# jean-pierreBoth/gsearch

Hardware: AMD Instinct MI355X
Metric: query genomes/sec (higher is better)
Workload: dtype f32

## Files before the change

### gsearch_amd/csrc/gs_index.hip

```cpp
#include <algorithm>
#include <functional>
#include <chrono>
#include <math.h>
#include <memory>
#include <stdlib.h>
#include <string.h>
#include <vector>
#include <sys/stat.h>
#include "gs_internal.hpp"
#include "gs_spec.hpp"
#include "gs_insert_rows.hpp"
#include "gs_hnswio_parse.hpp"

namespace gs {

constexpr int ST = 1024;
constexpr int SMAXI = 16;
constexpr int RIF = 8;
#define KEY(c, id) (((uint64_t)(c) << 32) | (uint64_t)(id))
#define KCNT(k) ((uint32_t)((k) >> 32))
#define KID(k) ((uint32_t)(k))
#define INF_CNT 0xFFFFFFFFu

struct IndexDev {
// ... 423 lines not shown
#pragma unroll
            for (int t = 0; t < 4; t++) if (top[t] && m >= (uint32_t)t) { const uint32_t c = m - t; atomicAdd(&coarse[c / HB], top[t]); if (c / HB == target) atomicAdd(&fine[c % HB], top[t]); }
        }
        __syncthreads();
        if (threadIdx.x < 64) {
            uint32_t run = 0, found = 0xFFFFFFFFu, before = 0;
            for (uint32_t b0 = 0; b0 < nb && found == 0xFFFFFFFFu; b0 += 64) {
                const uint32_t x = b0 + lane < nb ? coarse[b0 + lane] : 0;
                uint32_t inc = x;
#pragma unroll
                for (int o = 1; o < 64; o <<= 1) { const uint32_t y = __shfl_up(inc, o); if ((int)lane >= o) inc += y; }
                const uint64_t hit = __ballot(run + inc >= efs);
                if (hit) { const uint32_t l = (uint32_t)__ffsll((long long)hit) - 1; found = b0 + l; before = run + __shfl(inc, l) - __shfl(x, l); }
                run += __shfl(inc, 63);
            }
            if (lane == 0) { res[0] = found; res[1] = before; }
        }
        __syncthreads();
        const uint32_t bin = res[0], before = res[1];
        if (bin == target) {
            if (threadIdx.x == 0) { uint32_t run = before, f = 0; for (; f < (uint32_t)HB; f++) { run += fine[f]; if (run >= efs) break; } res[2] = bin * HB + f; }
            __syncthreads();
            const uint32_t tau = res[2];
            __syncthreads();
            return tau;
        }
        target = bin;
        __syncthreads();
    }
    return INF_CNT;
}

__device__ __forceinline__ uint32_t uni32(uint32_t v) { return (uint32_t)__builtin_amdgcn_readfirstlane((int)v); }
__device__ __forceinline__ uint32_t row_prefix4(uint32_t x)
{
    static_assert(DT / 64 == 8, "four wavefronts to a half of the workgroup");
    x += (uint32_t)__builtin_amdgcn_update_dpp(0, (int)x, 0x111, 0xF, 0xF, false);
    x += (uint32_t)__builtin_amdgcn_update_dpp(0, (int)x, 0x112, 0xF, 0xF, false);
    return x;
}

struct Phase2IO { uint32_t nT, evals, pops; bool tm; long long c_build, c_drain; uint64_t *wl; uint32_t cap_log, nlog; };
template <bool ONEG, bool WLOG, bool SPLIT>
__device__ __forceinline__ void dense_phase2(const IndexDev &ix, const DenseLds &S, uint32_t *vis, const uint16_t *__restrict__ matrow, uint32_t tau, uint32_t knbn,
                                                       uint64_t *Gold, uint64_t *Gnew, uint32_t headG, uint32_t nG, uint32_t headN, uint32_t nN, uint64_t Tmax, Phase2IO &io,
                                                       uint32_t vis_w, uint32_t *__restrict__ visg)
{
    const uint32_t maxdeg = 2 * ix.M;
    constexpr uint32_t CN = ONEG ? 512u : (uint32_t)DCN;
    const uint32_t wv = threadIdx.x >> 6, lane = threadIdx.x & 63;
    uint32_t nT = io.nT, st_p2 = 0;
    uint32_t *s_cnt = (uint32_t *)&S.scal[4];
    uint32_t *WL = (uint32_t *)Gnew;
    uint64_t *TA = Gold;
    if (threadIdx.x < 4) s_cnt[threadIdx.x] = threadIdx.x == 3 ? io.nlog : 0u;
    __syncthreads();
    {
        const uint64_t *src = Gold + headG;
        const uint32_t liveG = nG - headG, liveN = nN - headN;
        for (uint32_t i = threadIdx.x; i < liveG; i += DT) { const uint64_t k = src[i]; if (KCNT(k) <= tau) WL[atomicAdd(&s_cnt[0], 1u)] = KID(k); }
        for (uint32_t i = threadIdx.x; i < liveN; i += DT) { const uint64_t k = S.N[headN + i]; if (KCNT(k) <= tau) WL[atomicAdd(&s_cnt[0], 1u)] = KID(k); }
    }
    __syncthreads();
    uint32_t *bfA = (uint32_t *)S.A, *bfB = S.Eid;
    const uint32_t bytesA = 8 * maxdeg + 8 * (DWIN + 4) + 8 * (CN + 4), bytesB = (uint32_t)((uint8_t *)S.wsum - (uint8_t *)S.Eid);
    uint32_t lgA = 5, lgB = 5;
// ... 279 lines not shown
            }
        }
    }
    __syncthreads();
    for (uint32_t i0 = 0; i0 < n; i0 += NF * DT) {
        uint64_t kf[NF];
#pragma unroll
        for (int u = 0; u < NF; u++) { const uint32_t i = i0 + u * DT + threadIdx.x; kf[u] = i < n ? src[i] : ~(uint64_t)0; }
#pragma unroll
        for (int u = 0; u < NF; u++) {
            const uint64_t k = kf[u];
            const bool live = k != ~(uint64_t)0 && KCNT(k) <= dlimit;
            const bool isS = live && k < cutkey, isK = live && !isS;
            const uint64_t bS = __ballot(isS), bK = __ballot(isK);
            uint32_t baseS = 0, baseK = 0;
            if (lane == 0) { if (bS) baseS = atomicAdd(&cnt[0], (uint32_t)__popcll(bS)); if (bK) baseK = atomicAdd(&cnt[1], (uint32_t)__popcll(bK)); }
            baseS = (uint32_t)__builtin_amdgcn_readfirstlane((int)baseS); baseK = (uint32_t)__builtin_amdgcn_readfirstlane((int)baseK);
            if (isS) { const uint32_t pos = baseS + (uint32_t)__popcll(bS & ((1ull << lane) - 1)); if (pos < 64u) S.N[pos] = k; }
            if (isK) dst[baseK + (uint32_t)__popcll(bK & ((1ull << lane) - 1))] = k;
        }
    }
    __syncthreads();
    const uint32_t nsel = cnt[0] < 64u ? cnt[0] : 64u, nkeep = cnt[1];
    if (sel && wv == 0) {
        const uint64_t k = lane < nsel ? S.N[lane] : ~(uint64_t)0;
        uint32_t rank = 0;
        for (uint32_t j = 0; j < nsel; j++) rank += (S.N[j] < k);
        if (lane < nsel) S.N[64 + rank] = k;
    }
    __syncthreads();
    if (sel && wv == 0) {
        pkey = lane < nsel ? S.N[64 + lane] : ~(uint64_t)0;
        nP = nsel;
        pv = (nkeep && nsel) ? readlane_u64(pkey, (int)nsel - 1) : ~(uint64_t)0;
        if (lane < 3) S.W[fb + lane] = pkey;
    }
    if (threadIdx.x == 0) S.scal[4] = nkeep;
    stat += (sel ? 1ull : (1ull << 24)) + ((unsigned long long)rounds << 40);
    __syncthreads();
}

template <bool VLDS, bool PROF, int OCC, bool ONEG, bool WLOG, bool SPLIT = false>
__global__ __launch_bounds__(DT, OCC) void k_hnsw_search_dense(IndexDev ix, uint64_t nq, uint32_t knbn, uint32_t ef, const uint16_t *__restrict__ mat, uint64_t mat_ld,
                                                           uint32_t *__restrict__ scratch, uint32_t scratch_words, uint64_t *__restrict__ cbuf, uint32_t capC,
                                                           unsigned long long *__restrict__ counter, uint64_t *__restrict__ ids_out, float *__restrict__ dist_out,
                                                           uint32_t *__restrict__ count_out, uint64_t *__restrict__ evals_out, unsigned long long *__restrict__ prof,
                                                           unsigned long long *__restrict__ stats, uint64_t *__restrict__ wlog, uint32_t cap_log, uint32_t sort_cap,
                                                           uint64_t *__restrict__ w_out, uint32_t *__restrict__ w_n, const uint32_t *__restrict__ ep_in, uint32_t vis_w_arg)
{
    static_assert(!SPLIT || VLDS, "the split bitmap is a form of the LDS placement");
    extern __shared__ __attribute__((aligned(16))) uint8_t s_raw[];
    const uint32_t maxdeg = 2 * ix.M;
    const uint32_t efs = ef > knbn ? ef : knbn;
    const uint32_t vis_w = SPLIT ? vis_w_arg : 0u;
    const uint32_t nb = dense_nblocks(ix.m), hwords = nb * (HB / 2), vis_words = SPLIT ? (vis_w >> 5) : (uint32_t)((ix.n + 31) / 32);
    const uint32_t visg_words = SPLIT && ix.n > vis_w ? (uint32_t)((ix.n - vis_w + 31) / 32) : 0u;
    unsigned long long st_pq = 0;
    uint32_t st_pops = 0, st_acc = 0, st_p1 = 0, st_p2 = 0;
    constexpr bool PHASE2 = true;
#ifdef GS_DENSE_PQ_OFF
    constexpr bool PQ = false;
#else
    constexpr bool PQ = true;
#endif
    long long t_a = 0, t_b = 0, t_c = 0, t_d = 0, t_e = 0, n_pop = 0, n_merge = 0;
    long long tq1 = 0, tq2 = 0, tq3 = 0, tq4 = 0, tna = 0;
    constexpr uint32_t CN = ONEG ? 512u : (uint32_t)DCN;
    DenseLds S = carve_dense(s_raw, ix.m, knbn, maxdeg, SPLIT ? (uint64_t)vis_w : ix.n, VLDS, CN);
#define GS_TRAV_LOAD(p) __builtin_nontemporal_load(p)
#define GS_DROWX(K, PD, PI)                                                                                                \
    do {                                                                                                                   \
        const uint32_t rid_ = uni32(KID(K));                                                                               \
        uint32_t tx_ = threadIdx.x;                                                                                        \
        asm volatile("" : "+v"(tx_));                \
        const uint32_t hl_ = ONEG ? tx_ : tx_ & 255u, ho_ = hl_ * 4u;    \
        PD = ix.deg0[rid_];                                                                                                \
        PI = hl_ < maxdeg ? GS_TRAV_LOAD((const uint32_t *)((const uint8_t *)(ix.nbr0 + (uint64_t)rid_ * maxdeg) + ho_)) : 0; \
    } while (0)
#define GS_DROW(K) GS_DROWX(K, pdeg, pid)
    uint32_t *vis = VLDS ? S.vis : scratch + (uint64_t)blockIdx.x * scratch_words;
    Hist3 hs; hs.Hf = VLDS ? scratch + (uint64_t)blockIdx.x * scratch_words : S.Hf; hs.H2 = S.H2; hs.H1 = S.H1;
    uint32_t *visg = SPLIT ? scratch + (uint64_t)blockIdx.x * scratch_words + hwords : nullptr;
    uint64_t *Cb[2] = {cbuf + (uint64_t)blockIdx.x * 2 * capC, cbuf + (uint64_t)blockIdx.x * 2 * capC + capC};
    const uint32_t wv = threadIdx.x >> 6, lane = threadIdx.x & 63;
    const uint32_t half = ONEG ? 0u : threadIdx.x >> 8, hl = ONEG ? threadIdx.x : threadIdx.x & 255;
    for (;;) {
        __syncthreads();
        if (threadIdx.x == 0) S.scal[1] = atomicAdd(counter, 1ull);
        __syncthreads();
        const uint64_t qi = S.scal[1];
        if (qi >= nq) break;
        uint64_t *wl = WLOG ? wlog + (uint64_t)blockIdx.x * cap_log : nullptr;
        uint32_t nlog = 1;
        const uint16_t *matrow = mat + qi * mat_ld;
        const bool tm = PHASE2 && stats && blockIdx.x == 0 && threadIdx.x == 0;
        const long long tm0 = tm ? clock64() : 0;
        const uint32_t tau = PHASE2 ? dense_row_tau(matrow, ix.n, ix.m, efs, S.H1, S.hist, S.wsum) : 0u;
        const long long tm1 = tm ? clock64() : 0;
        for (uint32_t w = threadIdx.x; w < vis_words; w += DT) vis[w] = 0;
        if (SPLIT) for (uint32_t w = threadIdx.x; w < visg_words; w += DT) visg[w] = 0;
        for (uint32_t w = threadIdx.x; w < hwords; w += DT) hs.Hf[w] = 0;
        for (uint32_t w = threadIdx.x; w < nb * (HB / HG / 2); w += DT) S.H2[w] = 0;
        for (uint32_t w = threadIdx.x; w < nb; w += DT) S.H1[w] = 0;
        uint32_t evals = 1;
        uint32_t ep = (uint32_t)ix.entry, ep_cnt = matrow[ep];
        const bool given = WLOG && ep_in && ep_in[qi] != 0xFFFFFFFFu;
        if (given) { ep = ep_in[qi]; ep_cnt = matrow[ep]; evals = 0; }
        for (int L = given ? 0 : ix.top; L >= 1; L--) {
            for (;;) {
                const uint32_t *nbr; uint32_t deg;
                node_neighbours(ix, ep, L, nbr, deg);
                if (deg == 0) break;
                if (threadIdx.x == 0) S.scal[0] = ~(uint64_t)0;
                __syncthreads();
                evals += deg;
                if (threadIdx.x < deg) { const uint32_t c = matrow[nbr[threadIdx.x]]; if (c < ep_cnt) atomicMin((unsigned long long *)&S.scal[0], (unsigned long long)KEY(c, threadIdx.x)); }
// ... 40 lines not shown
                c = S.W[fb]; c1 = S.W[fb + 1]; c2 = S.W[fb + 2];
                const bool empty = c == ~(uint64_t)0, crowded = nU + maxdeg > capC && nU - nU_lc >= maxdeg;
                if (empty && nU == 0) break;
                if (empty || crowded) {
                    pq_rebuild(ix, S, Cb[cur], Cb[cur ^ 1], capC, nU, empty, full ? dmax : INF_CNT, pkey, pv, nP, fb, st_pq);
                    cur ^= 1; nU = (uint32_t)S.scal[4]; nU_lc = nU;
                    continue;
                }
                if (KCNT(c) > dmax) break;
                if (uni32(wv) == 0) {
                    pkey = wave_shl1_u64(pkey); if (lane == 63) pkey = ~(uint64_t)0;
                    nP--;
                    if (lane < 3) S.W[(fb ^ 4u) + lane] = pkey;
                }
            } else {
            if (headG < nG && headG - wbase >= wn) {
                __syncthreads();
                wbase = headG; wn = nG - headG < (uint32_t)DWIN ? nG - headG : (uint32_t)DWIN;
                if (threadIdx.x < wn + 3) S.W[threadIdx.x] = threadIdx.x < wn ? Cb[cur][headG + threadIdx.x] : ~(uint64_t)0;
                __syncthreads();
            }
            const uint32_t wo = headG - wbase;
            const uint64_t g0 = S.W[wo], g1 = S.W[wo + 1], g2 = S.W[wo + 2];
            const uint64_t n0 = S.N[headN], n1 = S.N[headN + 1], n2 = S.N[headN + 2];
            c = g0 < n0 ? g0 : n0;
            if (c == ~(uint64_t)0) break;
            if (KCNT(c) > dmax) break;
            if (g0 < n0) { headG++; c1 = g1 < n0 ? g1 : n0; c2 = g1 < n0 ? (g2 < n0 ? g2 : n0) : (g1 < n1 ? g1 : n1); }
            else { headN++; c1 = g0 < n1 ? g0 : n1; c2 = g0 < n1 ? (g1 < n1 ? g1 : n1) : (g0 < n2 ? g0 : n2); }
            }
            const long long p0 = PROF ? clock64() : 0;
            uint32_t id = 0, cntv = 0; bool unv = false, below = false;
            uint64_t bal = 0, balb = 0;
            const bool expanding = ONEG || uni32(half) == (it & 1u);
            if (expanding) {
                if (pk != c) {
                    if (ONEG && nk == c) { pid = nid; pdeg = ndeg; nk = ~(uint64_t)0; }
                    else GS_DROW(c);
                    pst = 1;
                }
                id = pid;
                if (hl < pdeg) {
                    const uint32_t bit = 1u << (id & 31);
                    uint32_t old;
                    if (SPLIT && id >= vis_w) {
                        if (pst == 2 && !pclr) old = bit;
                        else old = __hip_atomic_fetch_or(&visg[(id - vis_w) >> 5], bit, __ATOMIC_RELAXED, __HIP_MEMORY_SCOPE_WORKGROUP);
                    }
                    else if (VLDS) old = atomicOr(&vis[id >> 5], bit);
                    else old = __hip_atomic_fetch_or(&vis[id >> 5], bit, __ATOMIC_RELAXED, __HIP_MEMORY_SCOPE_WORKGROUP);
                    unv = !(old & bit);
                    if (unv) cntv = (pst == 2 && pclr) ? pcnt : (uint32_t)matrow[id];
                }
                below = unv && cntv < dmax;
                bal = __ballot(unv); balb = __ballot(below);
            } else if (!ONEG && c1 != ~(uint64_t)0) {
                if (pk != c1) {
                    pk = c1; pst = 1;
                    GS_DROW(c1);
                }
                if (VLDS) {
                    pclr = false;
                    if (hl < pdeg) {
                        if (SPLIT && pid >= vis_w) pclr = !((__hip_atomic_load(&visg[(pid - vis_w) >> 5], __ATOMIC_RELAXED, __HIP_MEMORY_SCOPE_AGENT) >> (pid & 31)) & 1u);
                        else pclr = !((vis[pid >> 5] >> (pid & 31)) & 1u);
                        if (pclr) pcnt = matrow[pid];
                    }
                    pst = 2;
                }
            } else if (!ONEG) pk = ~(uint64_t)0;
            it++;
            const long long p1 = PROF ? clock64() : 0;
            uint32_t *ws = S.wsum + ((it & 1) ? 8 : 0);
            if (expanding && lane == 0) ws[wv] = (uint32_t)__popcll(bal) | ((uint32_t)__popcll(balb) << 16);
            if (!ONEG) {
                if (expanding) {
                    pk = c2; pst = 1;
                    if (c2 != ~(uint64_t)0) GS_DROW(c2);
                }
            } else {
                pk = c1;
                if (c1 != ~(uint64_t)0) {
                    if (nk == c1) {
                        pid = nid; pdeg = ndeg; pclr = false;
                        if (VLDS) {
                            if (hl < pdeg) {
                                if (SPLIT && pid >= vis_w) pclr = !((__hip_atomic_load(&visg[(pid - vis_w) >> 5], __ATOMIC_RELAXED, __HIP_MEMORY_SCOPE_AGENT) >> (pid & 31)) & 1u);
                                else pclr = !((vis[pid >> 5] >> (pid & 31)) & 1u);
                                if (pclr) pcnt = matrow[pid];
                            }
                            pst = 2;
                        } else pst = 1;
                    } else { GS_DROW(c1); pst = 1; }
                }
                nk = c2;
                if (c2 != ~(uint64_t)0) GS_DROWX(c2, ndeg, nid);
            }
            lds_barrier();
            const long long p2 = PROF ? clock64() : 0;
            uint32_t tot = 0, pre = 0;
            if (ONEG) {
#pragma unroll
                for (int w = 0; w < DT / 64; w++) { const uint32_t x = ws[w]; tot += x; if (w < (int)wv) pre += x; }
            } else {
                const uint32_t wsw = ws[(((it & 1u) ^ 1u) << 2) + (lane & 3u)], wsum4 = row_prefix4(wsw);
                tot = (uint32_t)__builtin_amdgcn_readlane((int)wsum4, 3);
                pre = (uint32_t)__builtin_amdgcn_readlane((int)(wsum4 - wsw), (int)(uni32(wv) & 3u));
            }
            const uint32_t ne = tot & 0xFFFFu, B = tot >> 16;
            const long long p3 = PROF ? clock64() : 0;
            if (PROF && blockIdx.x == 0 && threadIdx.x == 0) { t_a += p1 - p0; t_b += p2 - p1; t_c += p3 - p2; n_pop++; }
            st_pops++;
            if (PHASE2 && dmax != tau) st_p1++;
            if (ne == 0) continue;
            evals += ne;
            bool slow;
            if (!full) slow = nR + ne > efs;
            else { if (B == 0) continue; slow = B > tieT; }
            uint64_t mykey = ~(uint64_t)0, ab; bool acc = false;
            uint32_t na, ci, aoff;
            const uint32_t off = pre & 0xFFFFu, boff = pre >> 16;
            if (!slow) { acc = below; na = B; ci = cntv; mykey = KEY(cntv, id); ab = balb; aoff = boff; }
            else {
                if (unv) { const uint32_t pos = off + (uint32_t)__popcll(bal & ((1ull << lane) - 1)); S.Eid[pos] = id; S.Ecnt[pos] = cntv; }
                const uint32_t CH = (nb + DT - 1) / DT;
                uint32_t loc = 0;
                for (uint32_t k2 = 0; k2 < CH; k2++) { const uint32_t idx = threadIdx.x * CH + k2; if (idx < nb) loc += S.H1[idx]; }
                uint32_t inc = loc;
#pragma unroll
                for (int o = 1; o < 64; o <<= 1) { const uint32_t y = __shfl_up(inc, o); if ((int)lane >= o) inc += y; }
                if (lane == 63) S.wsum[16 + wv] = inc;
                __syncthreads();
                ci = threadIdx.x < ne ? S.Ecnt[threadIdx.x] : INF_CNT;
                uint32_t woff = 0;
#pragma unroll
                for (int w = 0; w < DT / 64; w++) if (w < (int)wv) woff += S.wsum[16 + w];
                uint32_t run = woff + inc - loc;
                for (uint32_t k2 = 0; k2 < CH; k2++) { const uint32_t idx = threadIdx.x * CH + k2; if (idx < nb) { S.P1[idx] = run; run += S.H1[idx]; } }
                lds_barrier();
                if (threadIdx.x < ne && ci < dmax) {
                    uint32_t le = S.P1[ci / HB];
                    for (uint32_t g = (ci / HB) * (HB / HG); g < ci / HG; g++) le += h16(S.H2, g);
                    const uint32_t w0 = (ci / HG) * (HG / 2), w1 = ci >> 1;
                    for (uint32_t w = w0; w <= w1; w++) {
                        const uint32_t x = hf_word<VLDS>(hs.Hf, w);
                        le += x & 0xFFFFu;
                        if (w < w1 || (ci & 1)) le += x >> 16;
                    }
                    if (le < efs) {
#pragma unroll 8
                        for (uint32_t j = 0; j < threadIdx.x; j++) le += (S.Ecnt[j] <= ci);
                    }
                    acc = le < efs;
                }
                if (acc) mykey = KEY(ci, S.Eid[threadIdx.x]);
                ab = __ballot(acc);
                if (lane == 0) S.wsum[24 + wv] = (uint32_t)__popcll(ab);
                lds_barrier();
                aoff = 0; na = 0;
#pragma unroll
                for (int w = 0; w < DT / 64; w++) { const uint32_t x = S.wsum[24 + w]; if (w < (int)wv) aoff += x; na += x; }
            }
            const long long p4 = PROF ? clock64() : 0;
            if (PROF && blockIdx.x == 0 && threadIdx.x == 0) t_d += p4 - p3;
            if (na == 0) continue;
            n_merge++; st_acc++;
            uint64_t minA = 0;
            const uint32_t fbn = (it & 1u) * 4u;
            if (PQ) {
                if (acc) { hist_add<VLDS>(hs, ci, 1); S.As[aoff + (uint32_t)__popcll(ab & ((1ull << lane) - 1))] = mykey; }
                lds_barrier();
                if (uni32(wv) == 0) {
                    uint64_t tany = 0;
                    uint64_t *U = Cb[cur];
                    uint32_t nu = nU;
                    for (uint32_t b0 = 0; b0 < na; b0 += 64) {
                        const uint64_t k = b0 + lane < na ? S.As[b0 + lane] : ~(uint64_t)0;
                        tany |= __ballot(k < Tmax);
                        const bool toU = k != ~(uint64_t)0 && k >= pv;
                        const uint64_t bu = __ballot(toU);
                        if (toU) { const uint32_t pos = nu + (uint32_t)__popcll(bu & ((1ull << lane) - 1)); if (pos < capC) U[pos] = k; }
                        nu += (uint32_t)__popcll(bu);
                        uint64_t pend = __ballot(k != ~(uint64_t)0 && k < pv);
                        while (pend) {
                            const int l = __ffsll((long long)pend) - 1;
                            pend &= pend - 1;
                            const uint64_t kk = readlane_u64(k, l);
                            if (kk >= pv) { if (lane == 0 && nu < capC) U[nu] = kk; nu++; continue; }
                            const uint32_t pos = (uint32_t)__popcll(__ballot(pkey < kk));
                            const uint64_t ev = readlane_u64(pkey, 63), up = wave_shr1_u64(pkey);
                            pkey = lane < pos ? pkey : (lane == pos ? kk : up);
                            if (ev != ~(uint64_t)0) { if (lane == 0 && nu < capC) U[nu] = ev; nu++; }
                            else nP++;
                            if (nP == 64) pv = readlane_u64(pkey, 63);
                        }
                    }
                    if (lane < 3) S.W[fbn + lane] = pkey;
                    if (lane == 0) { S.scal[4] = nu; S.scal[5] = tany ? 0 : ~(uint64_t)0; }
                }
                lds_barrier();
                nU = (uint32_t)S.scal[4]; minA = S.scal[5];
            } else {
                if (acc) { hist_add<VLDS>(hs, ci, 1); S.As[aoff + (uint32_t)__popcll(ab & ((1ull << lane) - 1))] = mykey; }
                lds_barrier();
                if (threadIdx.x < na) {
                    const uint64_t k = S.As[threadIdx.x];
                    uint32_t rank = 0;
#pragma unroll 8
                    for (uint32_t j = 0; j < na; j++) rank += (S.As[j] < k);
                    S.A[rank] = k;
                }
                lds_barrier();
            }
            if (WLOG) { if (nlog + na <= cap_log && threadIdx.x < na) wl[nlog + threadIdx.x] = PQ ? S.As[threadIdx.x] : S.A[threadIdx.x]; nlog += na; }
            {
                const uint64_t a0 = PQ ? 0 : S.A[0], a1 = PQ ? 0 : (na > 1 ? S.A[1] : ~(uint64_t)0);
                const uint64_t n1 = PQ ? S.W[fbn] : (a0 < c1 ? a0 : c1);
                const uint64_t n2 = PQ ? S.W[fbn + 1] : (a0 < c1 ? (a1 < c1 ? a1 : c1) : (a0 < c2 ? a0 : c2));
                if (!ONEG) {
                    const uint64_t want = expanding ? n2 : n1;
                    if (want != ~(uint64_t)0 && pk != want) {
                        pk = want; pst = 1;
                        GS_DROW(want);
                    }
                } else {
                    if (n1 != ~(uint64_t)0 && pk != n1) {
                        const uint64_t ok = pk; const uint32_t oid = pid, odeg = pdeg;
                        if (nk == n1) { pid = nid; pdeg = ndeg; }
                        else GS_DROW(n1);
                        pk = n1; pst = 1;
                        nk = ok; nid = oid; ndeg = odeg;
                    }
                    if (n2 != ~(uint64_t)0 && nk != n2) { nk = n2; GS_DROWX(n2, ndeg, nid); }
                }
            }
            const long long q1 = PROF ? clock64() : 0;
            const uint32_t dold = dmax;
            if (nR + na >= efs) {
                const uint32_t excess = nR + na - efs;
                if (full && excess < tieT) {
                    if (threadIdx.x == 0 && excess) hist_sub<VLDS>(hs, dmax, excess);
                    tieT -= excess;
                } else {
                    __syncthreads();
                    if (threadIdx.x < 64) {
                        uint32_t d = full ? dmax : ix.m, ex = excess, tt = 0;
                        for (;;) {
                            d = hist_find_down<VLDS>(hs, d, lane, tt);
// ... 133 lines not shown
            uint32_t *cntp = (uint32_t *)s_raw;
            if (threadIdx.x == 0) cntp[0] = 0;
            __syncthreads();
            bool bad = nlog > cap_log;
            if (!bad) for (uint32_t i = threadIdx.x; i < nlog; i += DT) {
                const uint64_t k = wl[i];
                if (KCNT(k) <= dmax) { const uint32_t pos = atomicAdd(&cntp[0], 1u); if (pos < sort_cap) buf[pos] = k; }
            }
            __syncthreads();
            const uint32_t cnt = cntp[0];
            if (cnt > sort_cap) bad = true;
            if (bad) { if (threadIdx.x == 0) w_n[qi] = 0xFFFFFFFFu; }
            else {
                uint32_t n2 = 2; while (n2 < cnt) n2 <<= 1;
                for (uint32_t i = cnt + threadIdx.x; i < n2; i += DT) buf[i] = ~(uint64_t)0;
                __syncthreads();
                for (uint32_t kk = 2; kk <= n2; kk <<= 1)
                    for (uint32_t j = kk >> 1; j > 0; j >>= 1) {
                        for (uint32_t i = threadIdx.x; i < n2; i += DT) {
                            const uint32_t l = i ^ j;
                            if (l > i) {
                                const uint64_t a = buf[i], b = buf[l];
                                if ((a > b) == ((i & kk) == 0)) { buf[i] = b; buf[l] = a; }
                            }
                        }
                        __syncthreads();
                    }
                const uint32_t nW = cnt < efs ? cnt : efs;
                for (uint32_t i = threadIdx.x; i < nW; i += DT) w_out[qi * efs + i] = buf[i];
                if (threadIdx.x == 0) w_n[qi] = nW;
            }
        }
    }
#undef GS_DROW
#undef GS_DROWX
    if (stats && threadIdx.x == 0) { atomicAdd(&stats[1], (unsigned long long)st_pops); atomicAdd(&stats[2], (unsigned long long)st_acc); atomicAdd(&stats[5], (unsigned long long)st_p1); atomicAdd(&stats[6], (unsigned long long)st_p2); if (st_pq) atomicAdd(&stats[15], st_pq); }
    if (PROF && blockIdx.x == 0 && threadIdx.x == 0) {
        atomicAdd(&prof[0], (unsigned long long)t_a); atomicAdd(&prof[1], (unsigned long long)t_b); atomicAdd(&prof[2], (unsigned long long)t_c);
        atomicAdd(&prof[3], (unsigned long long)t_d); atomicAdd(&prof[4], (unsigned long long)t_e); atomicAdd(&prof[5], (unsigned long long)n_pop); atomicAdd(&prof[6], (unsigned long long)n_merge);
        atomicAdd(&prof[8], (unsigned long long)tq1); atomicAdd(&prof[9], (unsigned long long)tq2); atomicAdd(&prof[10], (unsigned long long)tq3); atomicAdd(&prof[11], (unsigned long long)tq4); atomicAdd(&prof[12], (unsigned long long)tna);
    }
}


__device__ __forceinline__ SearchLds carve_lds(uint8_t *base, uint32_t ef, uint32_t maxdeg)
{
    SearchLds S;
    const size_t capC = 2 * (size_t)ef + maxdeg + 64;
    S.R = (uint64_t *)base; base += 8 * (size_t)ef;
    S.C = (uint64_t *)base; base += 8 * capC;
    S.A = (uint64_t *)base; base += 8 * (size_t)maxdeg;
    S.As = (uint64_t *)base; base += 8 * (size_t)maxdeg;
    S.scal = (uint64_t *)base; base += 8 * 8;
    S.Eid = (uint32_t *)base; base += 4 * (size_t)maxdeg;
    S.Ecnt = (uint32_t *)base; base += 4 * (size_t)maxdeg;
    S.wsum = (uint32_t *)base;
    return S;
}

template <int KIND>
__global__ __launch_bounds__(ST) void k_hnsw_search(IndexDev ix, const uint8_t *__restrict__ queries, uint64_t nq, uint32_t knbn, uint32_t ef,
                                                     const uint16_t *__restrict__ mat, uint64_t mat_ld, uint32_t *__restrict__ visited, uint32_t vis_words, unsigned long long *__restrict__ counter,
                                                     uint64_t *__restrict__ ids_out, float *__restrict__ dist_out, uint32_t *__restrict__ count_out,
                                                     uint64_t *__restrict__ evals_out)
{
    extern __shared__ __attribute__((aligned(16))) uint8_t s_raw[];
    const uint32_t maxdeg = 2 * ix.M;
    const uint32_t efs = ef > knbn ? ef : knbn;
    SearchLds S = carve_lds(s_raw, efs, maxdeg);
// ... 830 lines not shown
{
    const size_t cap = 160 * 1024 - 1024;
    const size_t l = dense_lds_bytes(ix->prm.m, knbn, maxdeg, ix->n, true, maxdeg > (uint32_t)DT / 2 ? 512u : (uint32_t)DCN);
    const char *e = getenv("GS_DENSE_VIS");
    if (e && !strcmp(e, "global")) return false;
    if (e && !strcmp(e, "lds")) return l <= cap;
    return l <= cap;
}
static uint32_t dense_split_w(const gs_index *ix, uint32_t knbn, uint32_t maxdeg, uint32_t dcn, size_t min_bytes = 0, bool many_queries = false)
{
    const char *e = getenv("GS_DENSE_VIS");
    const bool forced = e && !strcmp(e, "split");
    if (e && !forced) { if (!strcmp(e, "global") || !strcmp(e, "lds")) return 0; }
    const bool one_per_cu = many_queries && round_up(dense_lds_bytes(ix->prm.m, knbn, maxdeg, ix->n, true, dcn), 1280) > (size_t)(160 * 1024 / 2);
    if (!forced && !one_per_cu && dense_vis_in_lds(ix, knbn, maxdeg)) return 0;
    const size_t base = std::max(dense_lds_bytes(ix->prm.m, knbn, maxdeg, 0, true, dcn), min_bytes);
    int per = getenv("GS_SPLIT_PER_CU") ? std::max(1, std::min(3, atoi(getenv("GS_SPLIT_PER_CU")))) : 2;
    uint64_t w = 0;
    for (; per >= 1 && w < 1024; per--) {
        const size_t budget = (size_t)(160 * 1024 / per) / 1280 * 1280 - 64;
        w = budget > base ? ((uint64_t)(budget - base) * 8) & ~(uint64_t)1023 : 0;
    }
    if (getenv("GS_SPLIT_W")) w = std::min<uint64_t>(w, (uint64_t)std::max(1024, atoi(getenv("GS_SPLIT_W"))) & ~(uint64_t)1023);
    if (w < 1024) return 0;
    return (uint32_t)std::min<uint64_t>(w, round_up(ix->n, 1024));
}
struct DenseGeom {
    bool ok;
    bool oneg, split, vlds;
    uint32_t dcn, vis_w;
    size_t lds;
    uint32_t per_cu, scratch_words, capC, grid;
    uint32_t p2_off;
};
static DenseGeom dense_geom(const gs_index *ix, uint64_t nq, uint32_t knbn, uint32_t ef, size_t min_lds_bytes, bool many_queries, bool with_log)
{
    const gs_ctx *c = ix->ctx;
    const size_t cap = 160 * 1024 - 1024;
    const uint32_t efs = std::max(ef, knbn), maxdeg = 2 * ix->prm.max_nb_conn;
    DenseGeom g{};
    g.oneg = maxdeg > (uint32_t)DT / 2;
    g.dcn = g.oneg ? 512u : (uint32_t)DCN;
    g.vis_w = dense_split_w(ix, knbn, maxdeg, g.dcn, min_lds_bytes, many_queries);
    g.split = g.vis_w != 0;
    const bool whole = dense_vis_in_lds(ix, knbn, maxdeg);
    g.vlds = with_log || g.split || whole;
    g.lds = std::max(dense_lds_bytes(ix->prm.m, knbn, maxdeg, g.split ? (uint64_t)g.vis_w : ix->n, g.vlds, g.dcn), min_lds_bytes);
    if (with_log && g.oneg) g.ok = false;
    else if (g.split) g.ok = true;
    else if (whole) g.ok = g.lds <= cap;
    else g.ok = !with_log && g.lds <= cap;
    const size_t granted = round_up(g.lds, 1280);
    g.per_cu = (uint32_t)std::max<size_t>(1, std::min<size_t>(3, (160 * 1024) / granted));
    if (g.oneg) g.per_cu = std::min<uint32_t>(g.per_cu, 2);
    if (!with_log && getenv("GS_DENSE_PER_CU")) g.per_cu = std::max(1, std::min((int)g.per_cu, atoi(getenv("GS_DENSE_PER_CU"))));
    g.scratch_words = (g.vlds ? dense_nblocks(ix->prm.m) * (HB / 2) : (uint32_t)((ix->n + 31) / 32)) + (g.split && ix->n > g.vis_w ? (uint32_t)((ix->n - g.vis_w + 31) / 32) : 0u);
    g.capC = 2 * efs + 2 * g.dcn + maxdeg + 64;
    g.grid = (uint32_t)std::min<uint64_t>(nq, (uint64_t)c->n_cu * g.per_cu);
    g.p2_off = (getenv("GS_DENSE_PHASE2") && !atoi(getenv("GS_DENSE_PHASE2"))) ? 1u : 0u;
    return g;
}
static int search_launch_dense(gs_index *ix, uint64_t nq, uint32_t knbn, uint32_t ef, const uint16_t *mat, uint64_t mat_ld, uint64_t *ids, float *dist,
                               uint32_t *count, uint64_t *evals)
{
    gs_ctx *c = ix->ctx;
    const DenseGeom g = dense_geom(ix, nq, knbn, ef, 0, nq >= (uint64_t)2 * c->n_cu, false);
    int rc;
    if ((rc = ensure_stats(ix))) return rc;
    ix->stat_wg_in_flight = g.grid; ix->stat_adj_row_bytes = (uint64_t)8 * ix->prm.max_nb_conn + 4;
    if ((rc = ix->visited.ensure((size_t)4 * g.scratch_words * c->n_cu * 3))) return rc;
    if ((rc = ix->cbuf.ensure((size_t)16 * g.capC * c->n_cu * 3))) return rc;
    GS_HIP_CHECK(hipMemsetAsync(ix->counter.p, 0, 8, c->stream));
    IndexDev d = index_dev(ix);
    unsigned long long *prof = nullptr;
    DevBuf profbuf;
    if (getenv("GS_TRAV_PROFILE")) { if ((rc = profbuf.alloc(128))) return rc; GS_HIP_CHECK(hipMemsetAsync(profbuf.p, 0, 128, c->stream)); prof = profbuf.as<unsigned long long>(); }
    {
    ProfScope ps(c, FAM_SEARCH);
#define GS_LAUNCH_DSEARCH(V, P, O, G) GS_LAUNCH_DSEARCH_S(V, P, O, G, false)
#define GS_LAUNCH_DSEARCH_S(V, P, O, G, SP)                                                                                  \
    do {                                                                                                                  \
        auto kern = k_hnsw_search_dense<V, P, O, G, false, SP>;                                                            \
        GS_HIP_CHECK(hipFuncSetAttribute((const void *)kern, hipFuncAttributeMaxDynamicSharedMemorySize, (int)g.lds));    \
        hipLaunchKernelGGL(kern, dim3(g.grid), dim3(DT), g.lds, c->stream, d, nq, knbn, ef, mat, mat_ld, ix->visited.as<uint32_t>(), g.scratch_words, \
                           ix->cbuf.as<uint64_t>(), g.capC, ix->counter.as<unsigned long long>(), ids, dist, count, evals, prof, ix->stats.as<unsigned long long>(),  \
                           (uint64_t *)nullptr, g.p2_off, 0u, (uint64_t *)nullptr, (uint32_t *)nullptr, (const uint32_t *)nullptr, g.vis_w);  \
    } while (0)
    if (g.split) { if (g.oneg) GS_LAUNCH_DSEARCH_S(true, false, 4, true, true); else GS_LAUNCH_DSEARCH_S(true, false, 4, false, true); }
    else if (g.oneg) { if (g.vlds) GS_LAUNCH_DSEARCH(true, false, 4, true); else GS_LAUNCH_DSEARCH(false, false, 4, true); }
    else if (prof) { if (g.vlds) GS_LAUNCH_DSEARCH(true, true, 4, false); else GS_LAUNCH_DSEARCH(false, true, 4, false); }
    else if (g.per_cu >= 3) { if (g.vlds) GS_LAUNCH_DSEARCH(true, false, 6, false); else GS_LAUNCH_DSEARCH(false, false, 6, false); }
    else { if (g.vlds) GS_LAUNCH_DSEARCH(true, false, 4, false); else GS_LAUNCH_DSEARCH(false, false, 4, false); }
#undef GS_LAUNCH_DSEARCH
#undef GS_LAUNCH_DSEARCH_S
    }
    GS_HIP_CHECK(hipGetLastError());
    if (prof) {
        unsigned long long h[16];
        GS_HIP_CHECK(hipMemcpyAsync(h, prof, 128, hipMemcpyDeviceToHost, c->stream));
        GS_HIP_CHECK(hipStreamSynchronize(c->stream));
        fprintf(stderr, "[GS_TRAV_PROFILE] workgroup 0: pops %llu merges %llu | cycles/pop: loads+atomics issue->ballot %.0f, sync1 %.0f, compaction+sync2 %.0f, accept rule+count %.0f | merge cycles/merge %.0f\n",
                h[5], h[6], (double)h[0] / h[5], (double)h[1] / h[5], (double)h[2] / h[5], (double)h[3] / h[5], h[6] ? (double)h[4] / h[6] : 0.0);
        if (h[6]) fprintf(stderr, "[GS_TRAV_PROFILE] of %llu accepting pops: %llu merged into T, %llu folded N into G\n", h[6], h[13], h[14]);
        if (h[6]) fprintf(stderr, "[GS_TRAV_PROFILE] per accepting pop: compaction+sort %.0f, prefetch+trim %.0f, T %.0f, fold+N merge %.0f cycles; accepted keys %.2f\n",
                          (double)h[8] / h[6], (double)h[9] / h[6], (double)h[10] / h[6], (double)h[11] / h[6], (double)h[12] / h[6]);
    }
    return GS_OK;
}

static bool dense_traversal_fits(const gs_index *ix, uint32_t knbn, uint32_t efs)
{
    const uint32_t maxdeg = 2 * ix->prm.max_nb_conn;
    return maxdeg <= (uint32_t)DT && efs <= 65535u && knbn <= (uint32_t)(TMAXI * DT) && ix->prm.m <= 65535u &&
           dense_lds_bytes(ix->prm.m, knbn, maxdeg, ix->n, false, maxdeg > (uint32_t)DT / 2 ? 512u : (uint32_t)DCN) <= 160 * 1024 - 1024 && !getenv("GS_DENSE_LEGACY");
}
static int search_launch(gs_index *ix, const uint8_t *q_padded_dev, uint64_t nq, uint32_t knbn, uint32_t ef, const uint16_t *mat, uint64_t mat_ld,
                         uint64_t *ids, float *dist, uint32_t *count, uint64_t *evals)
{
    gs_ctx *c = ix->ctx;
// ... 133 lines not shown
    ix->user_rowbytes = gs::kind_bytes(p->kind) * (size_t)p->m;
    ix->stride = gs::round_up(ix->rowbytes, 256);
    ix->nchunks = (uint32_t)((ix->rowbytes + 15) / 16);
    *out = ix;
    return GS_OK;
}
void gs_index_destroy(gs_index *ix)
{
    if (!ix) return;
    GS_CTX_LOCK(ix->ctx);
    (void)hipSetDevice(ix->ctx->device);
    (void)hipStreamSynchronize(ix->ctx->stream);
    delete ix;
}
uint64_t gs_index_nb_point(const gs_index *ix) { return ix ? ix->n : 0; }
int gs_index_search_stats(gs_index *ix, uint64_t out[8], int reset)
{
    GS_REQUIRE(ix && out, GS_ERR_INVALID, "null argument");
    gs_ctx *c = ix->ctx;
    GS_CTX_LOCK(c);
    for (int i = 0; i < 8; i++) out[i] = 0;
    if (ix->stats.p) {
        GS_HIP_CHECK(hipSetDevice(c->device));
        unsigned long long h[16];
        GS_HIP_CHECK(hipMemcpyAsync(h, ix->stats.p, 128, hipMemcpyDeviceToHost, c->stream));
        if (reset) GS_HIP_CHECK(hipMemsetAsync(ix->stats.p, 0, 128, c->stream));
        GS_HIP_CHECK(hipStreamSynchronize(c->stream));
        out[0] = h[0]; out[1] = h[1]; out[2] = h[2]; out[5] = h[5]; out[6] = h[6]; out[7] = h[7];
        if (getenv("GS_TRAV_PHASES") && h[12])
            fprintf(stderr, "[GS_TRAV_PHASES] workgroup 0, %llu queries: cycles per query tau scan %.0f, phase 1 %.0f, phase 2 %.0f, output %.0f\n", h[12],
                    (double)h[8] / h[12], (double)h[9] / h[12], (double)h[10] / h[12], (double)h[11] / h[12]),
            fprintf(stderr, "[GS_TRAV_PHASES]   inside phase 2: work list + Bloom build %.0f, drain %.0f, merge into T %.0f\n", (double)h[13] / h[12], (double)h[14] / h[12],
                    ((double)h[10] - (double)h[13] - (double)h[14]) / h[12]),
            fprintf(stderr, "[GS_TRAV_PHASES]   phase 1 front, all workgroups: refills %llu, compactions %llu, selection rounds beyond the first %llu\n", h[15] & 0xFFFFFFull, (h[15] >> 24) & 0xFFFFull, h[15] >> 40);
    }
    out[3] = ix->stat_wg_in_flight; out[4] = ix->stat_adj_row_bytes;
    return GS_OK;
}
int gs_index_debug_fill_scratch(gs_index *ix, int byte)
{
    GS_REQUIRE(ix && byte >= 0 && byte <= 255, GS_ERR_INVALID, "gs_index_debug_fill_scratch: null index or byte outside 0..255");
    GS_CTX_LOCK(ix->ctx);
    GS_HIP_CHECK(hipDeviceSynchronize());
    for (gs::DevBuf *b : gs::index_scratch(ix)) if (b->p) GS_HIP_CHECK(hipMemset(b->p, byte, b->bytes));
    GS_HIP_CHECK(hipDeviceSynchronize());
    return GS_OK;
}
int gs_index_release_build_scratch(gs_index *ix)
{
    GS_REQUIRE(ix, GS_ERR_INVALID, "gs_index_release_build_scratch: null index");
    GS_CTX_LOCK(ix->ctx);
    const uint64_t budget = ix->pair_cache_budget;
    gs::drop_pair_cache(ix);
    ix->pair_cache_budget = budget;
    return GS_OK;
}
uint64_t gs_index_insert_evals(const gs_index *ix) { return ix ? ix->insert_evals : 0; }
int gs_index_get_params(const gs_index *ix, gs_index_params *out)
{
    GS_REQUIRE(ix && out, GS_ERR_INVALID, "null argument");
    *out = ix->prm;
    return GS_OK;
}

int gs_index_import(gs_index *ix, const void *sigs, uint64_t n, const uint8_t *levels, int64_t entry, const uint32_t *deg0,
                    const uint32_t *nbr0, const uint32_t *cnt0, const int32_t *upidx, uint64_t n_upper, const uint32_t *degU,
                    const uint32_t *nbrU, const uint32_t *cntU)
// ... 347 lines not shown
{
    if (ix->n < 4096 || ix->entry < 0 || efc > 65535u || efc < 2 || ix->prm.m > 65535u) return false;
    pg->sort_cap = 2; while (pg->sort_cap < 4 * efc) pg->sort_cap <<= 1;
    pg->g = dense_geom(ix, nb, 1, efc, (size_t)8 * pg->sort_cap + 64, false, true);
    return pg->g.ok;
}
static int plan_prepass(gs_index *ix, const PrepassGeom &pg, uint32_t nb, uint32_t efc, const uint16_t *mat, uint64_t mat_ld, const uint64_t **w0k, const uint32_t **w0n,
                        const uint64_t **w0e)
{
    gs_ctx *c = ix->ctx;
    *w0k = nullptr; *w0n = nullptr; *w0e = nullptr;
    const DenseGeom &g = pg.g;
    const uint32_t knbn = 1, cap_log = 16 * efc + g.p2_off;
    int rc;
    if ((rc = ensure_stats(ix))) return rc;
    if ((rc = ix->visited.ensure((size_t)4 * g.scratch_words * c->n_cu * 3))) return rc;
    if ((rc = ix->cbuf.ensure((size_t)16 * g.capC * c->n_cu * 3))) return rc;
    if ((rc = ix->counter.ensure(64))) return rc;
    if ((rc = ix->wlog.ensure((size_t)8 * cap_log * g.grid))) return rc;
    if ((rc = ix->w0_keys.ensure((size_t)8 * efc * nb))) return rc;
    if ((rc = ix->w0_n.ensure((size_t)4 * nb))) return rc;
    if ((rc = ix->w0_evals.ensure((size_t)8 * nb))) return rc;
    GS_HIP_CHECK(hipMemsetAsync(ix->counter.p, 0, 8, c->stream));
    IndexDev d = index_dev(ix);
    {
#define GS_LAUNCH_WL(O) GS_LAUNCH_WL_S(O, false)
#define GS_LAUNCH_WL_S(O, SP)                                                                                             \
    do {                                                                                                                  \
        auto kern = k_hnsw_search_dense<true, false, O, false, true, SP>;                                                 \
        GS_HIP_CHECK(hipFuncSetAttribute((const void *)kern, hipFuncAttributeMaxDynamicSharedMemorySize, (int)g.lds));    \
        hipLaunchKernelGGL(kern, dim3(g.grid), dim3(DT), g.lds, c->stream, d, (uint64_t)nb, knbn, efc, mat, mat_ld, ix->visited.as<uint32_t>(), g.scratch_words, \
                           ix->cbuf.as<uint64_t>(), g.capC, ix->counter.as<unsigned long long>(), (uint64_t *)nullptr, (float *)nullptr, (uint32_t *)nullptr, \
                           ix->w0_evals.as<uint64_t>(), (unsigned long long *)nullptr, (unsigned long long *)nullptr, ix->wlog.as<uint64_t>(), cap_log, pg.sort_cap, \
                           ix->w0_keys.as<uint64_t>(), ix->w0_n.as<uint32_t>(), ix->ep0.as<uint32_t>(), g.vis_w);             \
    } while (0)
        if (g.split) GS_LAUNCH_WL_S(4, true); else if (g.per_cu >= 3) GS_LAUNCH_WL(6); else GS_LAUNCH_WL(4);
#undef GS_LAUNCH_WL
#undef GS_LAUNCH_WL_S
    }
    GS_HIP_CHECK(hipGetLastError());
    *w0k = ix->w0_keys.as<uint64_t>(); *w0n = ix->w0_n.as<uint32_t>(); *w0e = ix->w0_evals.as<uint64_t>();
    return GS_OK;
}
}

namespace {
struct InsertEnv {
    const char *pair_cache_gb = getenv("GS_PAIR_CACHE_GB");
    const char *sparse_rows = getenv("GS_SPARSE_ROWS"), *sparse_l = getenv("GS_SPARSE_L"), *sparse_arena_gb = getenv("GS_SPARSE_ARENA_GB"),
               *sparse_bitmap_gb = getenv("GS_SPARSE_BITMAP_GB"), *sparse_chunk_mb = getenv("GS_SPARSE_ARENA_CHUNK_MB");
    uint32_t group = 8;
    bool prepass = !(getenv("GS_PLAN_PREPASS") && !atoi(getenv("GS_PLAN_PREPASS")));
    bool plan_vis_global = getenv("GS_PLAN_VIS_GLOBAL") != nullptr, sparse_verbose = getenv("GS_SPARSE_VERBOSE") != nullptr;
    InsertEnv() { if (const char *e = getenv("GS_INSERT_GROUP")) group = (uint32_t)std::max(1, std::min(12, atoi(e))); }
};

struct InsertCall {
    gs_index *ix; gs_ctx *c; uint64_t n;
    const InsertEnv env;
    const uint32_t M, ML, maxdeg, efc, B, ef_lds;
    const size_t lds;
    const bool cnt16;
    uint64_t first = 0, slab_ld = 0;
    std::vector<uint8_t> lv; std::vector<int32_t> up;
    bool appended = false;
    uint32_t ext_cap = 0;
    gs::GraphDev g;
// ... 646 lines not shown
```

Before: 51650.

## Add direct append path for accepting pops that cannot touch the priority queue

```diff
diff --git a/gsearch_amd/csrc/gs_index.hip b/gsearch_amd/csrc/gs_index.hip
--- a/gsearch_amd/csrc/gs_index.hip
+++ b/gsearch_amd/csrc/gs_index.hip
@@ -479,6 +479,7 @@
 }
 
 __device__ __forceinline__ uint32_t uni32(uint32_t v) { return (uint32_t)__builtin_amdgcn_readfirstlane((int)v); }
+__device__ __forceinline__ uint64_t uni64(uint64_t v) { return (uint64_t)uni32((uint32_t)v) | ((uint64_t)uni32((uint32_t)(v >> 32)) << 32); }
 __device__ __forceinline__ uint32_t row_prefix4(uint32_t x)
 {
     static_assert(DT / 64 == 8, "four wavefronts to a half of the workgroup");
@@ -824,9 +825,9 @@
     if (sel && wv == 0) {
         pkey = lane < nsel ? S.N[64 + lane] : ~(uint64_t)0;
         nP = nsel;
-        pv = (nkeep && nsel) ? readlane_u64(pkey, (int)nsel - 1) : ~(uint64_t)0;
         if (lane < 3) S.W[fb + lane] = pkey;
     }
+    if (sel) pv = (nkeep && nsel) ? uni64(S.N[64 + nsel - 1]) : ~(uint64_t)0;
     if (threadIdx.x == 0) S.scal[4] = nkeep;
     stat += (sel ? 1ull : (1ull << 24)) + ((unsigned long long)rounds << 40);
     __syncthreads();
@@ -838,7 +839,7 @@
                                                            unsigned long long *__restrict__ counter, uint64_t *__restrict__ ids_out, float *__restrict__ dist_out,
                                                            uint32_t *__restrict__ count_out, uint64_t *__restrict__ evals_out, unsigned long long *__restrict__ prof,
                                                            unsigned long long *__restrict__ stats, uint64_t *__restrict__ wlog, uint32_t cap_log, uint32_t sort_cap,
-                                                           uint64_t *__restrict__ w_out, uint32_t *__restrict__ w_n, const uint32_t *__restrict__ ep_in, uint32_t vis_w_arg)
+                                                           uint64_t *__restrict__ w_out, uint32_t *__restrict__ w_n, const uint32_t *__restrict__ ep_in, uint32_t vis_w_arg, uint32_t direct_off)
 {
     static_assert(!SPLIT || VLDS, "the split bitmap is a form of the LDS placement");
     extern __shared__ __attribute__((aligned(16))) uint8_t s_raw[];
@@ -848,7 +849,7 @@
     const uint32_t nb = dense_nblocks(ix.m), hwords = nb * (HB / 2), vis_words = SPLIT ? (vis_w >> 5) : (uint32_t)((ix.n + 31) / 32);
     const uint32_t visg_words = SPLIT && ix.n > vis_w ? (uint32_t)((ix.n - vis_w + 31) / 32) : 0u;
     unsigned long long st_pq = 0;
-    uint32_t st_pops = 0, st_acc = 0, st_p1 = 0, st_p2 = 0;
+    uint32_t st_pops = 0, st_acc = 0, st_p1 = 0, st_p2 = 0, st_dir = 0;
     constexpr bool PHASE2 = true;
 #ifdef GS_DENSE_PQ_OFF
     constexpr bool PQ = false;
@@ -874,6 +875,7 @@
     Hist3 hs; hs.Hf = VLDS ? scratch + (uint64_t)blockIdx.x * scratch_words : S.Hf; hs.H2 = S.H2; hs.H1 = S.H1;
     uint32_t *visg = SPLIT ? scratch + (uint64_t)blockIdx.x * scratch_words + hwords : nullptr;
     uint64_t *Cb[2] = {cbuf + (uint64_t)blockIdx.x * 2 * capC, cbuf + (uint64_t)blockIdx.x * 2 * capC + capC};
+#define GS_U_APPEND(CUR) (cbuf + ((uint64_t)blockIdx.x * 2 * capC + ((CUR) ? capC : 0u)))
     const uint32_t wv = threadIdx.x >> 6, lane = threadIdx.x & 63;
     const uint32_t half = ONEG ? 0u : threadIdx.x >> 8, hl = ONEG ? threadIdx.x : threadIdx.x & 255;
     for (;;) {
@@ -980,6 +982,7 @@
             const long long p0 = PROF ? clock64() : 0;
             uint32_t id = 0, cntv = 0; bool unv = false, below = false;
             uint64_t bal = 0, balb = 0;
+            uint32_t cflag = 0;
             const bool expanding = ONEG || uni32(half) == (it & 1u);
             if (expanding) {
                 if (pk != c) {
@@ -1002,6 +1005,10 @@
                 }
                 below = unv && cntv < dmax;
                 bal = __ballot(unv); balb = __ballot(below);
+                if (PQ) {
+                    if (direct_off || nT != knbn) cflag = 0x1000u;
+                    else { const uint64_t fence = pv > Tmax ? pv : Tmax; cflag = (__ballot(KEY(cntv, id) < fence) & balb) ? 0x1000u : 0u; }
+                }
             } else if (!ONEG && c1 != ~(uint64_t)0) {
                 if (pk != c1) {
                     pk = c1; pst = 1;
@@ -1020,7 +1027,7 @@
             it++;
             const long long p1 = PROF ? clock64() : 0;
             uint32_t *ws = S.wsum + ((it & 1) ? 8 : 0);
-            if (expanding && lane == 0) ws[wv] = (uint32_t)__popcll(bal) | ((uint32_t)__popcll(balb) << 16);
+            if (expanding && lane == 0) ws[wv] = (uint32_t)__popcll(bal) | ((uint32_t)__popcll(balb) << 16) | cflag;
             if (!ONEG) {
                 if (expanding) {
                     pk = c2; pst = 1;
@@ -1055,7 +1062,7 @@
                 tot = (uint32_t)__builtin_amdgcn_readlane((int)wsum4, 3);
                 pre = (uint32_t)__builtin_amdgcn_readlane((int)(wsum4 - wsw), (int)(uni32(wv) & 3u));
             }
-            const uint32_t ne = tot & 0xFFFFu, B = tot >> 16;
+            const uint32_t ne = tot & 0xFFFu, B = tot >> 16;
             const long long p3 = PROF ? clock64() : 0;
             if (PROF && blockIdx.x == 0 && threadIdx.x == 0) { t_a += p1 - p0; t_b += p2 - p1; t_c += p3 - p2; n_pop++; }
             st_pops++;
@@ -1067,7 +1074,7 @@
             else { if (B == 0) continue; slow = B > tieT; }
             uint64_t mykey = ~(uint64_t)0, ab; bool acc = false;
             uint32_t na, ci, aoff;
-            const uint32_t off = pre & 0xFFFFu, boff = pre >> 16;
+            const uint32_t off = pre & 0xFFFu, boff = pre >> 16;
             if (!slow) { acc = below; na = B; ci = cntv; mykey = KEY(cntv, id); ab = balb; aoff = boff; }
             else {
                 if (unv) { const uint32_t pos = off + (uint32_t)__popcll(bal & ((1ull << lane) - 1)); S.Eid[pos] = id; S.Ecnt[pos] = cntv; }
@@ -1115,12 +1122,23 @@
             n_merge++; st_acc++;
             uint64_t minA = 0;
             const uint32_t fbn = (it & 1u) * 4u;
-            if (PQ) {
+            const bool direct = PQ && !slow && !(tot & 0xF000u);
+            if (direct) {
+                st_dir++;
+                if (acc) {
+                    hist_add<VLDS>(hs, ci, 1);
+                    const uint32_t r = aoff + (uint32_t)__popcll(ab & ((1ull << lane) - 1));
+                    if (nU + r < capC) GS_U_APPEND(cur)[nU + r] = mykey;
+                    if (WLOG && nlog + na <= cap_log) wl[nlog + r] = mykey;
+                }
+                nU += na; minA = ~(uint64_t)0;
+                if (WLOG) nlog += na;
+            } else if (PQ) {
                 if (acc) { hist_add<VLDS>(hs, ci, 1); S.As[aoff + (uint32_t)__popcll(ab & ((1ull << lane) - 1))] = mykey; }
                 lds_barrier();
                 if (uni32(wv) == 0) {
                     uint64_t tany = 0;
-                    uint64_t *U = Cb[cur];
+                    uint64_t *U = GS_U_APPEND(cur);
                     uint32_t nu = nU;
                     for (uint32_t b0 = 0; b0 < na; b0 += 64) {
                         const uint64_t k = b0 + lane < na ? S.As[b0 + lane] : ~(uint64_t)0;
@@ -1144,10 +1162,10 @@
                         }
                     }
                     if (lane < 3) S.W[fbn + lane] = pkey;
-                    if (lane == 0) { S.scal[4] = nu; S.scal[5] = tany ? 0 : ~(uint64_t)0; }
+                    if (lane == 0) { S.scal[4] = nu; S.scal[5] = tany ? 0 : ~(uint64_t)0; S.scal[7] = pv; }
                 }
                 lds_barrier();
-                nU = (uint32_t)S.scal[4]; minA = S.scal[5];
+                nU = (uint32_t)S.scal[4]; minA = S.scal[5]; pv = uni64(S.scal[7]);
             } else {
                 if (acc) { hist_add<VLDS>(hs, ci, 1); S.As[aoff + (uint32_t)__popcll(ab & ((1ull << lane) - 1))] = mykey; }
                 lds_barrier();
@@ -1160,8 +1178,8 @@
                 }
                 lds_barrier();
             }
-            if (WLOG) { if (nlog + na <= cap_log && threadIdx.x < na) wl[nlog + threadIdx.x] = PQ ? S.As[threadIdx.x] : S.A[threadIdx.x]; nlog += na; }
-            {
+            if (WLOG && !direct) { if (nlog + na <= cap_log && threadIdx.x < na) wl[nlog + threadIdx.x] = PQ ? S.As[threadIdx.x] : S.A[threadIdx.x]; nlog += na; }
+            if (!direct) {
                 const uint64_t a0 = PQ ? 0 : S.A[0], a1 = PQ ? 0 : (na > 1 ? S.A[1] : ~(uint64_t)0);
                 const uint64_t n1 = PQ ? S.W[fbn] : (a0 < c1 ? a0 : c1);
                 const uint64_t n2 = PQ ? S.W[fbn + 1] : (a0 < c1 ? (a1 < c1 ? a1 : c1) : (a0 < c2 ? a0 : c2));
@@ -1361,9 +1379,10 @@
             }
         }
     }
+#undef GS_U_APPEND
 #undef GS_DROW
 #undef GS_DROWX
-    if (stats && threadIdx.x == 0) { atomicAdd(&stats[1], (unsigned long long)st_pops); atomicAdd(&stats[2], (unsigned long long)st_acc); atomicAdd(&stats[5], (unsigned long long)st_p1); atomicAdd(&stats[6], (unsigned long long)st_p2); if (st_pq) atomicAdd(&stats[15], st_pq); }
+    if (stats && threadIdx.x == 0) { atomicAdd(&stats[1], (unsigned long long)st_pops); atomicAdd(&stats[2], (unsigned long long)st_acc); if (st_dir) atomicAdd(&stats[3], (unsigned long long)st_dir); atomicAdd(&stats[5], (unsigned long long)st_p1); atomicAdd(&stats[6], (unsigned long long)st_p2); if (st_pq) atomicAdd(&stats[15], st_pq); }
     if (PROF && blockIdx.x == 0 && threadIdx.x == 0) {
         atomicAdd(&prof[0], (unsigned long long)t_a); atomicAdd(&prof[1], (unsigned long long)t_b); atomicAdd(&prof[2], (unsigned long long)t_c);
         atomicAdd(&prof[3], (unsigned long long)t_d); atomicAdd(&prof[4], (unsigned long long)t_e); atomicAdd(&prof[5], (unsigned long long)n_pop); atomicAdd(&prof[6], (unsigned long long)n_merge);
@@ -2260,6 +2279,7 @@
     size_t lds;
     uint32_t per_cu, scratch_words, capC, grid;
     uint32_t p2_off;
+    uint32_t direct_off;
 };
 static DenseGeom dense_geom(const gs_index *ix, uint64_t nq, uint32_t knbn, uint32_t ef, size_t min_lds_bytes, bool many_queries, bool with_log)
 {
@@ -2286,6 +2306,7 @@
     g.capC = 2 * efs + 2 * g.dcn + maxdeg + 64;
     g.grid = (uint32_t)std::min<uint64_t>(nq, (uint64_t)c->n_cu * g.per_cu);
     g.p2_off = (getenv("GS_DENSE_PHASE2") && !atoi(getenv("GS_DENSE_PHASE2"))) ? 1u : 0u;
+    g.direct_off = (getenv("GS_DENSE_DIRECT") && !atoi(getenv("GS_DENSE_DIRECT"))) ? 1u : 0u;
     return g;
 }
 static int search_launch_dense(gs_index *ix, uint64_t nq, uint32_t knbn, uint32_t ef, const uint16_t *mat, uint64_t mat_ld, uint64_t *ids, float *dist,
@@ -2312,7 +2333,7 @@
         GS_HIP_CHECK(hipFuncSetAttribute((const void *)kern, hipFuncAttributeMaxDynamicSharedMemorySize, (int)g.lds));    \
         hipLaunchKernelGGL(kern, dim3(g.grid), dim3(DT), g.lds, c->stream, d, nq, knbn, ef, mat, mat_ld, ix->visited.as<uint32_t>(), g.scratch_words, \
                            ix->cbuf.as<uint64_t>(), g.capC, ix->counter.as<unsigned long long>(), ids, dist, count, evals, prof, ix->stats.as<unsigned long long>(),  \
-                           (uint64_t *)nullptr, g.p2_off, 0u, (uint64_t *)nullptr, (uint32_t *)nullptr, (const uint32_t *)nullptr, g.vis_w);  \
+                           (uint64_t *)nullptr, g.p2_off, 0u, (uint64_t *)nullptr, (uint32_t *)nullptr, (const uint32_t *)nullptr, g.vis_w, g.direct_off);  \
     } while (0)
     if (g.split) { if (g.oneg) GS_LAUNCH_DSEARCH_S(true, false, 4, true, true); else GS_LAUNCH_DSEARCH_S(true, false, 4, false, true); }
     else if (g.oneg) { if (g.vlds) GS_LAUNCH_DSEARCH(true, false, 4, true); else GS_LAUNCH_DSEARCH(false, false, 4, true); }
@@ -2512,7 +2533,8 @@
                     (double)h[8] / h[12], (double)h[9] / h[12], (double)h[10] / h[12], (double)h[11] / h[12]),
             fprintf(stderr, "[GS_TRAV_PHASES]   inside phase 2: work list + Bloom build %.0f, drain %.0f, merge into T %.0f\n", (double)h[13] / h[12], (double)h[14] / h[12],
                     ((double)h[10] - (double)h[13] - (double)h[14]) / h[12]),
-            fprintf(stderr, "[GS_TRAV_PHASES]   phase 1 front, all workgroups: refills %llu, compactions %llu, selection rounds beyond the first %llu\n", h[15] & 0xFFFFFFull, (h[15] >> 24) & 0xFFFFull, h[15] >> 40);
+            fprintf(stderr, "[GS_TRAV_PHASES]   phase 1 front, all workgroups: refills %llu, compactions %llu, selection rounds beyond the first %llu\n", h[15] & 0xFFFFFFull, (h[15] >> 24) & 0xFFFFull, h[15] >> 40),
+            fprintf(stderr, "[GS_TRAV_PHASES]   phase 1 hand-over, all workgroups: accepting pops %llu, direct %llu\n", h[2], h[3]);
     }
     out[3] = ix->stat_wg_in_flight; out[4] = ix->stat_adj_row_bytes;
     return GS_OK;
@@ -2926,7 +2948,7 @@
         hipLaunchKernelGGL(kern, dim3(g.grid), dim3(DT), g.lds, c->stream, d, (uint64_t)nb, knbn, efc, mat, mat_ld, ix->visited.as<uint32_t>(), g.scratch_words, \
                            ix->cbuf.as<uint64_t>(), g.capC, ix->counter.as<unsigned long long>(), (uint64_t *)nullptr, (float *)nullptr, (uint32_t *)nullptr, \
                            ix->w0_evals.as<uint64_t>(), (unsigned long long *)nullptr, (unsigned long long *)nullptr, ix->wlog.as<uint64_t>(), cap_log, pg.sort_cap, \
-                           ix->w0_keys.as<uint64_t>(), ix->w0_n.as<uint32_t>(), ix->ep0.as<uint32_t>(), g.vis_w);             \
+                           ix->w0_keys.as<uint64_t>(), ix->w0_n.as<uint32_t>(), ix->ep0.as<uint32_t>(), g.vis_w, g.direct_off); \
     } while (0)
         if (g.split) GS_LAUNCH_WL_S(4, true); else if (g.per_cu >= 3) GS_LAUNCH_WL(6); else GS_LAUNCH_WL(4);
 #undef GS_LAUNCH_WL
```

After: 51890, median of 6. No clear change (+0.5%).
